# NagsTheProgrammer/WindGNN

Hardware: NVIDIA B200
Metric: gcn_gru_forward_sequences_per_s (higher is better)
Workload: dtype f32

## Files before the change

### windgnn_b200/csrc/abi.cu

```cuda

#include "../../include/windgnn_b200.h"

#include <cmath>
#include <cstdarg>
#include <cstdio>
#include <cstdlib>
#include <cstring>
#include <mutex>
#include <vector>

#include "gcn.cuh"
#include "gcn_bwd.cuh"
#include "gcn_bwd_rows.cuh"
#include "gcn_rows.cuh"
#include "gcn_sparse.cuh"
#include "gcn_sparse_plan.cuh"
#include "gemm_kb.cuh"
#include "gru_bwd.cuh"
#include "inproj.cuh"
#include "inproj_tc2.cuh"
#include "recur.cuh"
#include "recur_tc.cuh"
#include "recur_unit.cuh"
#include "sgemm.cuh"
#include "train_misc.cuh"
#include "wg_common.cuh"

namespace {

thread_local char g_err[512] = "";

int fail(int code, const char* fmt, ...) {
    va_list ap;
    va_start(ap, fmt);
    vsnprintf(g_err, sizeof(g_err), fmt, ap);
    va_end(ap);
    return code;
}

#define WG_CUDA(expr)                                                                          \
    do {                                                                                       \
        cudaError_t e_ = (expr);                                                               \
        if (e_ != cudaSuccess)                                                                 \
            return fail(WG_ERR_CUDA, "%s failed: %s (%s:%d)", #expr, cudaGetErrorString(e_),   \
                        __FILE__, __LINE__);                                                   \
    } while (0)

struct DeviceGuard {
    int prev = -1;
    cudaError_t err = cudaSuccess;
    explicit DeviceGuard(int dev) {
        err = cudaGetDevice(&prev);
        if (err == cudaSuccess && prev != dev) err = cudaSetDevice(dev);
    }
    ~DeviceGuard() {
        int cur = -1;
        if (prev >= 0 && cudaGetDevice(&cur) == cudaSuccess && cur != prev) cudaSetDevice(prev);
    }
};

constexpr size_t kAlign = 256;
size_t align_up(size_t v) { return (v + kAlign - 1) / kAlign * kAlign; }

enum GcnKind { kGcnRows, kGcn13x7, kGcn13x4, kGcn16x4, kGcnSparsePlan, kGcnSparseLanes };
enum RecurKind { kRecurTc, kRecurUnit, kRecurWide };

struct Plan {
    int T, S, Fi, Fh, Fo, H;
    long long chunk;
    int I, G;
    int IP;
    int NPB;
    int GP;
    int KP;
    int NPR;
    int n_bias;
    bool sparse;
    GcnKind gcn;
    size_t gcn_smem;
    int gcn_rb;
    int gcn_threads;
    size_t off_sqw, off_sqsteps, off_sqpairs;
    bool tc;
    wg::Tc2Shape tc2;
    RecurKind recur;
    bool regw;
    bool whu;
    int ru_wpg, ru_ht;
    int ru_rmax;
    int rc_ts;
    size_t rc_smem;
    size_t off_wp, off_bias, off_wht, off_whu, off_bhn, off_u, off_gi, off_z, total;
    size_t off_whh_hi, off_whh_lo;
};

long long default_chunk(long long B, size_t bytes_per_seq) {
    long long c = (long long)wg::kNumSMs * wg::kRcBT;
    const size_t cap = (size_t)6 << 30;
    if ((size_t)c * bytes_per_seq > cap) {
        c = (long long)(cap / bytes_per_seq) / wg::kRcBT * wg::kRcBT;
        if (c < wg::kRcBT) c = wg::kRcBT;
    }
    return B < c ? (B < 1 ? 1 : B) : c;
}

GcnKind dense_gcn_kind(int S, int Fi, int Fh, int Fo) {
    if (Fi == 13 && Fh == 13 && Fo == 13) return wg::ceil_div(S, 7) * 7 <= wg::ceil_div(S, 4) * 4 ? kGcn13x7 : kGcn13x4;
    return kGcn16x4;
}

int dense_gcn_geometry(GcnKind k, int S, int Fi, int Fh, int Fo, int& RB, size_t& smem) {
    const int Fmax = Fi > Fh ? (Fi > Fo ? Fi : Fo) : (Fh > Fo ? Fh : Fo);
    if (Fmax > 16) return fail(WG_ERR_UNSUPPORTED, "GCN feature width %d > 16 is not built into the dense kernel", Fmax);
    const int NSG = wg::ceil_div(S, k == kGcn13x7 ? 7 : 4);
    if (NSG > wg::kGcnThreads)
        return fail(WG_ERR_UNSUPPORTED, "S=%d too large for the dense GCN kernel", S);
    auto smem_of = [&](int rb) {
        const size_t floats = k == kGcn13x7   ? wg::gcn_smem_floats<13, 7>(S, Fmax, rb)
                              : k == kGcn13x4 ? wg::gcn_smem_floats<13, 4>(S, Fmax, rb)
                                              : wg::gcn_smem_floats<16, 4>(S, Fmax, rb);
        return floats * 4;
    };
    RB = wg::kGcnThreads / NSG;
    const int in_cols = S * Fi;
    const int need = (in_cols % 4 == 0) ? 1 : (in_cols % 2 == 0 ? 2 : 4);
    if (RB > need) RB -= RB % need;
    smem = smem_of(RB);
    while (smem > (size_t)wg::kMaxSmemOptin / 3 && RB > 2 * need && RB > 8) {
        RB -= need > (RB + 7) / 8 ? need : (RB + 7) / 8 / need * need;
        smem = smem_of(RB);
    }
    while (smem > (size_t)wg::kMaxSmemOptin && RB > 1) {
        RB = RB / 2;
        smem = smem_of(RB);
    }
    if (smem > (size_t)wg::kMaxSmemOptin)
        return fail(WG_ERR_UNSUPPORTED, "dense GCN needs %zu B of shared memory (S=%d); use the sparse path", smem, S);
    return WG_OK;
}

bool force_legacy() {
    const char* e = getenv("WG_FORCE_LEGACY");
    return e && e[0] == '1';
}

long long forecast_piece_rows(const Plan& p, long long Ttot) {
    const long long r = p.chunk * p.T;
    return r < Ttot ? r : Ttot;
}

int plan_layout(Plan& p, long long B, int T, int S, int Fi, int Fh, int Fo, int H, long long chunk, bool sparse,
                int flags, long long table_rows = 0) {
    if (B < 0 || T <= 0 || S <= 0 || Fi <= 0 || Fh <= 0 || Fo <= 0 || H <= 0 || chunk < 0)
        return fail(WG_ERR_BAD_ARG, "non-positive dimension (B=%lld T=%d S=%d F=%d/%d/%d H=%d chunk=%lld)",
                    B, T, S, Fi, Fh, Fo, H, chunk);
    if ((long long)S * Fo > (1 << 20) || H > (1 << 15))
        return fail(WG_ERR_UNSUPPORTED, "dimension too large (S*F_out=%lld, H=%d)", (long long)S * Fo, H);
    p.T = T; p.S = S; p.Fi = Fi; p.Fh = Fh; p.Fo = Fo; p.H = H;
    p.sparse = sparse;
    if (flags & ~WG_FLAG_TENSOR_CORES) return fail(WG_ERR_BAD_ARG, "unknown flags 0x%x", flags);
    p.I = S * Fo;
    p.G = 3 * H;
    p.tc2 = wg::tc2_shape(p.G, p.I);
    p.tc = (flags & WG_FLAG_TENSOR_CORES) != 0;
    if (p.tc && !p.tc2.ok)
        return fail(WG_ERR_UNSUPPORTED, "tensor-core projection: unsupported gate width 3H = %d", p.G);
    p.IP = p.tc ? p.tc2.KP : wg::round_up(p.I, wg::kIpBK);
    p.NPB = wg::round_up(p.G, wg::kIpBN);
    p.GP = wg::round_up(p.G, 8);
    p.KP = wg::round_up(H, 4);
    p.NPR = wg::recur_np(p.G);
    {
        const size_t per_seq = (size_t)T * ((size_t)p.IP + p.GP + (sparse ? (size_t)S * Fo : 0)) * 4;
        p.chunk = chunk > 0 ? chunk : default_chunk(B, per_seq);
        if (p.chunk > B && B > 0) p.chunk = B;
    }
    if (sparse)
        p.gcn = Fi <= wg::kSpF && Fo <= wg::kSpF && Fh <= wg::kSqMaxFh &&
                        wg::gcn_sparse_plan_smem_bytes(S, Fi, Fo) <= (size_t)wg::kMaxSmemOptin
                    ? kGcnSparsePlan : kGcnSparseLanes;
    else if (wg::gcn_rows_applies(S, Fi, Fh, Fo) && wg::gcn_rows_smem_floats(S) * 4 <= (size_t)wg::kMaxSmemOptin &&
             !force_legacy())
        p.gcn = kGcnRows;
    else
        p.gcn = dense_gcn_kind(S, Fi, Fh, Fo);
    p.whu = wg::recur_u_applies(H);
    if (p.tc && wg::recur_tc_applies(H) && wg::recur_tc_smem_bytes(H) <= (size_t)wg::kMaxSmemOptin)
        p.recur = kRecurTc;
    else if (p.whu && wg::recur_u_smem_floats(H, wg::kRuMinR) * 4 <= (size_t)wg::kMaxSmemOptin)
        p.recur = kRecurUnit;
    else
        p.recur = kRecurWide;
    p.regw = (p.KP == 104 || p.KP == 24) && p.NPR <= wg::kRwThreads &&
             wg::recur_regw_smem_floats(p.KP, p.NPR, p.GP) * 4 <= (size_t)wg::kMaxSmemOptin;
    p.ru_wpg = wg::recur_u_wpg(H);
    p.ru_ht = H == 102 || H == 21 ? H : 0;
    size_t o = 0;
    const int wrows = p.tc && p.tc2.NP > p.NPB ? p.tc2.NP : p.NPB;
    p.n_bias = wrows > 512 ? wrows : 512;
    p.off_wp = o;   o = align_up(o + (p.tc ? wg::tc2_w_halves(p.tc2) * 2 : (size_t)p.NPB * p.IP * 4));
    p.off_bias = o; o = align_up(o + (size_t)p.n_bias * 4);
    p.off_wht = o;  o = align_up(o + (size_t)p.KP * p.NPR * 4);
    p.off_whu = o;
    if (p.whu) o = align_up(o + (size_t)p.KP * 3 * wg::recur_u_hp2(H) * 4);
    p.off_bhn = o;  o = align_up(o + (size_t)p.KP * 4);
    const bool tc_recur = p.recur == kRecurTc;
    p.off_whh_hi = o; if (tc_recur) o = align_up(o + wg::recur_tc_w_halves(H) * 2);
    p.off_whh_lo = o; if (tc_recur) o = align_up(o + wg::recur_tc_w_halves(H) * 2);
    const size_t rows = table_rows > 0 ? (size_t)forecast_piece_rows(p, table_rows) : (size_t)p.chunk * T;
    const size_t rows_tiled = (rows + wg::kUTileRows - 1) / wg::kUTileRows * wg::kUTileRows;
    p.off_u = o;    o = align_up(o + rows_tiled * p.IP * 4);
    const size_t rows_gi =
        table_rows > 0 ? (size_t)table_rows : (size_t)((p.chunk + wg::kRtSeqs - 1) / wg::kRtSeqs * wg::kRtSeqs) * T;
    p.off_gi = o;   o = align_up(o + rows_gi * p.GP * 4);
    p.off_z = o;    if (sparse) o = align_up(o + (rows + wg::kNumSMs) * (size_t)S * Fo * 4);
    const bool sq = p.gcn == kGcnSparsePlan;
    p.off_sqw = o;     if (sq) o = align_up(o + sizeof(wg::SqWeights));
    p.off_sqsteps = o;
    p.off_sqpairs = o + (size_t)wg::round_up(wg::ceil_div(S, 32), 4) * sizeof(int);
    if (sq) o = align_up(o + wg::sq_plan_bytes(S));
    p.total = o;
    return WG_OK;
}

int plan_launch(Plan& p) {
    const long long rows = p.chunk * p.T;
    switch (p.gcn) {
    case kGcnRows:
        p.gcn_smem = wg::gcn_rows_smem_floats(p.S) * 4;
        p.gcn_threads = wg::gcn_rows_warps(p.S) * 32;
        break;
    case kGcnSparsePlan: {
        p.gcn_smem = wg::gcn_sparse_plan_smem_bytes(p.S, p.Fi, p.Fo);
        const long long rt = (rows + wg::kSpThreads - 1) / wg::kSpThreads * wg::kSpThreads;
        if (rt / 32 > 65535) return fail(WG_ERR_UNSUPPORTED, "sparse GCN: chunk of %lld rows too large", rows);
        break;
    }
    case kGcnSparseLanes:
        if (p.Fi > wg::kSpF || p.Fo > wg::kSpF)
            return fail(WG_ERR_UNSUPPORTED, "sparse GCN: F_in / F_out must be <= %d (got %d / %d)", wg::kSpF, p.Fi, p.Fo);
        p.gcn_smem = ((size_t)2 * p.Fh * wg::kSpF + p.Fh) * 4;
        if (p.gcn_smem > (size_t)wg::kMaxSmemOptin)
            return fail(WG_ERR_UNSUPPORTED, "sparse GCN: hidden width %d too large", p.Fh);
        break;
    default: {
        const int rc = dense_gcn_geometry(p.gcn, p.S, p.Fi, p.Fh, p.Fo, p.gcn_rb, p.gcn_smem);
        if (rc) return rc;
    }
    }
    if (!p.tc && (rows + wg::kIpBM - 1) / wg::kIpBM * (p.NPB / wg::kIpBN) > 0x7fffffffLL)
        return fail(WG_ERR_UNSUPPORTED, "projection grid too large");
    if (p.recur == kRecurUnit) {
        p.ru_rmax = wg::kRuMaxR;
        while (p.ru_rmax > wg::kRuMinR && wg::recur_u_smem_floats(p.H, p.ru_rmax) * 4 > (size_t)wg::kMaxSmemOptin)
            --p.ru_rmax;
    } else if (p.recur == kRecurWide) {
        p.rc_ts = wg::recur_stage_steps(p.H);
        p.rc_smem = wg::recur_smem_floats(p.KP, p.GP, p.H, p.rc_ts) * 4;
        if (p.rc_smem > (size_t)wg::kMaxSmemOptin) {
            p.rc_ts = 0;
            p.rc_smem = wg::recur_smem_floats(p.KP, p.GP) * 4;
        }
        if (p.rc_smem > (size_t)wg::kMaxSmemOptin)
            return fail(WG_ERR_UNSUPPORTED, "GRU hidden size %d: state does not fit shared memory", p.H);
    }
    return WG_OK;
}

int make_plan(Plan& p, long long B, int T, int S, int Fi, int Fh, int Fo, int H, long long chunk,
              bool sparse = false, int flags = 0) {
    const int rc = plan_layout(p, B, T, S, Fi, Fh, Fo, H, chunk, sparse, flags);
    return rc ? rc : plan_launch(p);
}

int check_ws(const void* ws, size_t bytes, size_t need) {
    if (!ws) return fail(WG_ERR_WORKSPACE, "workspace is NULL (need %zu bytes)", need);
    if (reinterpret_cast<uintptr_t>(ws) % kAlign)
        return fail(WG_ERR_WORKSPACE, "workspace must be %zu-byte aligned", kAlign);
    if (bytes < need)
        return fail(WG_ERR_WORKSPACE, "workspace too small: %zu bytes given, %zu needed", bytes, need);
    return WG_OK;
}

template <typename T>
T* ws_ptr(void* ws, size_t off) { return reinterpret_cast<T*>(static_cast<char*>(ws) + off); }

__global__ void pack_params_kernel(const float* __restrict__ w_ih, const float* __restrict__ w_hh,
                                   const float* __restrict__ b_ih, const float* __restrict__ b_hh,
                                   float* __restrict__ wp, float* __restrict__ bias,
                                   float* __restrict__ wht, float* __restrict__ whu, float* __restrict__ bhn, int I,
                                   int H, int IP, int NPB, int KP, int NPR, int pack_wih, int n_bias) {
    const int G = 3 * H;
    const long long n_wp = pack_wih ? (long long)NPB * IP : 0;
    const long long n_wht = (long long)KP * NPR;
    const long long stride = (long long)gridDim.x * blockDim.x;
    const long long t0 = (long long)blockIdx.x * blockDim.x + threadIdx.x;
    for (long long e = t0; e < n_wp; e += stride) {
        const int nl = (int)(e % wg::kIpBN);
        const long long r = e / wg::kIpBN;
        const int k = (int)(r % IP), n = (int)(r / IP) * wg::kIpBN + nl;
        wp[e] = (n < G && k < I) ? w_ih[(size_t)n * I + k] : 0.0f;
    }
    for (long long e = t0; e < n_wht; e += stride) {
        const int k = (int)(e / NPR), n = (int)(e % NPR);
        wht[e] = (k < H && n < G) ? w_hh[(size_t)n * H + k] : 0.0f;
    }
    if (whu != nullptr) {
        const int HP2 = wg::recur_u_hp2(H);
        const long long n_whu = (long long)KP * 3 * HP2;
        for (long long e = t0; e < n_whu; e += stride) {
            const int j = (int)(e % HP2);
            const long long r = e / HP2;
            const int g = (int)(r % 3), k = (int)(r / 3);
            whu[e] = (k < H && j < H) ? w_hh[((size_t)g * H + j) * H + k] : 0.0f;
        }
    }
    for (long long e = t0; e < n_bias; e += stride) {
        float v = 0.0f;
        if (e < G) v = b_ih[e] + (e < 2 * H ? b_hh[e] : 0.0f);
        bias[e] = v;
    }
    for (long long e = t0; e < KP; e += stride) bhn[e] = e < H ? b_hh[2 * H + e] : 0.0f;
}

template <int FP, int SG, bool EXACT, int LAYERS, bool TILED>
int launch_gcn_t(const float* X, const float* adj, const float* W1, const float* b1, const float* W2,
                 const float* b2, float* out, long long R, int S, int Fi, int Fh, int Fo, int ldo, int RB, size_t smem,
                 cudaStream_t st) {
    auto kern = wg::gcn_kernel<FP, SG, EXACT, LAYERS, TILED>;
    WG_CUDA(cudaFuncSetAttribute(kern, cudaFuncAttributeMaxDynamicSharedMemorySize, (int)smem));
    int per_sm = 0;
    WG_CUDA(cudaOccupancyMaxActiveBlocksPerMultiprocessor(&per_sm, kern, wg::kGcnThreads, smem));
    if (per_sm < 1) per_sm = 1;
    const long long nblocks = (R + RB - 1) / RB;
    long long grid = (long long)wg::kNumSMs * per_sm;
    if (grid > nblocks) grid = nblocks;
    if (grid < 1) return WG_OK;
    kern<<<(unsigned)grid, wg::kGcnThreads, smem, st>>>(X, adj, W1, b1, W2, b2, out, R, S, Fi, Fh, Fo, ldo, RB);
    WG_CUDA(cudaGetLastError());
    return WG_OK;
}

template <int LAYERS, bool TILED>
int launch_gcn_dense(GcnKind k, int RB, size_t smem, const float* X, const float* adj, const float* W1,
                     const float* b1, const float* W2, const float* b2, float* out, long long R, int S, int Fi, int Fh,
                     int Fo, int ldo, cudaStream_t st) {
#define WG_GCN(FP, SG, EX) \
    launch_gcn_t<FP, SG, EX, LAYERS, TILED>(X, adj, W1, b1, W2, b2, out, R, S, Fi, Fh, Fo, ldo, RB, smem, st)
    if (k == kGcn13x7) return WG_GCN(13, 7, true);
    if (k == kGcn13x4) return WG_GCN(13, 4, true);
    return WG_GCN(16, 4, false);
#undef WG_GCN
}

int launch_gcn_rows(const Plan& p, const float* X, const float* adj, const float* W1, const float* b1,
                    const float* W2, const float* b2, float* out, long long R, cudaStream_t st) {
    WG_CUDA(cudaFuncSetAttribute(wg::gcn_rows_kernel, cudaFuncAttributeMaxDynamicSharedMemorySize, (int)p.gcn_smem));
    int per_sm = 0;
    WG_CUDA(cudaOccupancyMaxActiveBlocksPerMultiprocessor(&per_sm, wg::gcn_rows_kernel, p.gcn_threads, p.gcn_smem));
    if (per_sm < 1) per_sm = 1;
    const long long nblocks = (R + wg::kGrRows - 1) / wg::kGrRows;
    long long grid = (long long)wg::kNumSMs * per_sm;
    if (grid > nblocks) grid = nblocks;
    if (grid < 1) return WG_OK;
    wg::gcn_rows_kernel<<<(unsigned)grid, p.gcn_threads, p.gcn_smem, st>>>(X, adj, W1, b1, W2, b2, out, R, p.S, p.IP);
    WG_CUDA(cudaGetLastError());
    return WG_OK;
}

struct Graph {
    const float* adj;
    const int* rowptr;
    const int* colidx;
    const float* vals;
};

int launch_gcn_sparse(const Plan& p, void* ws, const Graph& g, const float* x, const float* w1, const float* b1,
                      const float* w2, const float* b2, long long rows, cudaStream_t st) {
    if (rows < 1) return WG_OK;
    if (p.gcn == kGcnSparsePlan) {
        const bool narrow = p.Fi <= 13 && p.Fo <= 13, exact = p.Fi == 13 && p.Fo == 13;
        auto kern = exact ? wg::gcn_sparse_plan_kernel<13, true>
                          : narrow ? wg::gcn_sparse_plan_kernel<13, false> : wg::gcn_sparse_plan_kernel<16, false>;
        WG_CUDA(cudaFuncSetAttribute(kern, cudaFuncAttributeMaxDynamicSharedMemorySize, (int)p.gcn_smem));
        const unsigned grid = (unsigned)(rows < wg::kNumSMs ? rows : wg::kNumSMs);
        float* urow = ws_ptr<float>(ws, p.off_z);
        float* zscr = urow + (size_t)rows * p.S * p.Fo;
        kern<<<grid, wg::kSqThreads, p.gcn_smem, st>>>(x, g.rowptr, g.colidx, g.vals, ws_ptr<int>(ws, p.off_sqsteps),
                                                       ws_ptr<int2>(ws, p.off_sqpairs), zscr, urow, rows, p.S, p.Fi,
                                                       p.Fh, p.Fo);
        WG_CUDA(cudaGetLastError());
        const long long rt = (rows + wg::kSpThreads - 1) / wg::kSpThreads * wg::kSpThreads;
        const dim3 tg((unsigned)((p.S + 31) / 32), (unsigned)(rt / 32));
        const size_t tsmem = wg::fmajor_to_tiles_smem_bytes(p.Fo);
        WG_CUDA(cudaFuncSetAttribute(wg::fmajor_to_tiles_kernel, cudaFuncAttributeMaxDynamicSharedMemorySize, (int)tsmem));
        wg::fmajor_to_tiles_kernel<<<tg, 256, tsmem, st>>>(urow, ws_ptr<float>(ws, p.off_u), rows, p.S, p.Fo, p.IP);
        WG_CUDA(cudaGetLastError());
        return WG_OK;
    }
    const long long tiles = (rows + wg::kSpThreads - 1) / wg::kSpThreads;
    int chunks = (int)((4LL * wg::kNumSMs * 4 + tiles - 1) / tiles);
    if (chunks < 1) chunks = 1;
    if (chunks > p.S) chunks = p.S;
    const int s_chunk = (p.S + chunks - 1) / chunks;
    const dim3 grid((unsigned)tiles, (unsigned)((p.S + s_chunk - 1) / s_chunk));
    WG_CUDA(cudaFuncSetAttribute(wg::gcn_sparse_l1_kernel, cudaFuncAttributeMaxDynamicSharedMemorySize,
                                 (int)p.gcn_smem));
    wg::gcn_sparse_l1_kernel<<<grid, wg::kSpThreads, p.gcn_smem, st>>>(x, g.rowptr, g.colidx, g.vals, w1, b1, w2,
                                                                       ws_ptr<float>(ws, p.off_z), rows, p.S, p.Fi,
                                                                       p.Fh, p.Fo, s_chunk);
    WG_CUDA(cudaGetLastError());
    wg::gcn_sparse_l2_kernel<<<grid, wg::kSpThreads, 0, st>>>(ws_ptr<float>(ws, p.off_z), g.rowptr, g.colidx, g.vals,
                                                             b2, ws_ptr<float>(ws, p.off_u), rows, p.S, p.Fo, p.IP,
                                                             s_chunk);
    WG_CUDA(cudaGetLastError());
    return WG_OK;
}

int launch_gcn(const Plan& p, void* ws, const Graph& g, const float* x, const float* w1, const float* b1,
               const float* w2, const float* b2, long long rows, cudaStream_t st) {
    float* u = ws_ptr<float>(ws, p.off_u);
    if (p.gcn == kGcnRows) return launch_gcn_rows(p, x, g.adj, w1, b1, w2, b2, u, rows, st);
    if (p.sparse) return launch_gcn_sparse(p, ws, g, x, w1, b1, w2, b2, rows, st);
    return launch_gcn_dense<2, true>(p.gcn, p.gcn_rb, p.gcn_smem, x, g.adj, w1, b1, w2, b2, u, rows, p.S, p.Fi, p.Fh,
                                     p.Fo, p.IP, st);
}

int launch_inproj_tc(const Plan& p, void* ws, long long rows, cudaStream_t st, float* gi) {
    const long long m_tiles = (rows + wg::kT2BM - 1) / wg::kT2BM;
    if (m_tiles < 1) return WG_OK;
    const wg::Tc2Shape& t = p.tc2;
    WG_CUDA(cudaFuncSetAttribute(wg::inproj_tc2_kernel, cudaFuncAttributeMaxDynamicSharedMemorySize,
                                 (int)t.smem_bytes));
    const long long tiles = m_tiles * t.n_nt;
    const unsigned grid = (unsigned)(tiles < wg::kNumSMs ? tiles : wg::kNumSMs);
    wg::inproj_tc2_kernel<<<grid, wg::kT2Threads, t.smem_bytes, st>>>(
        ws_ptr<float>(ws, p.off_u), ws_ptr<__half>(ws, p.off_wp), ws_ptr<float>(ws, p.off_bias), gi, rows, p.IP,
        t.KP, p.GP, t.n_nt, t.N_each, t.stages);
    WG_CUDA(cudaGetLastError());
    return WG_OK;
}

int launch_inproj(const Plan& p, void* ws, long long rows, cudaStream_t st, float* gi) {
    if (p.tc) return launch_inproj_tc(p, ws, rows, st, gi);
    const long long m_tiles = (rows + wg::kIpBM - 1) / wg::kIpBM;
    const int n_tiles = p.NPB / wg::kIpBN;
    const long long grid = m_tiles * n_tiles;
    if (grid < 1) return WG_OK;
    WG_CUDA(cudaFuncSetAttribute(wg::inproj_kernel, cudaFuncAttributeMaxDynamicSharedMemorySize,
                                 wg::kIpSmemBytes));
    wg::inproj_kernel<<<(unsigned)grid, wg::kIpThreads, wg::kIpSmemBytes, st>>>(
        ws_ptr<float>(ws, p.off_u), ws_ptr<float>(ws, p.off_wp), ws_ptr<float>(ws, p.off_bias), gi, rows, p.IP, p.GP,
        n_tiles);
    WG_CUDA(cudaGetLastError());
    return WG_OK;
}


int launch_recur_wide(const Plan& p, void* ws, float* out, long long Bc, cudaStream_t st, const long long* row0) {
    auto kern = row0 ? wg::gru_recur_kernel<true> : wg::gru_recur_kernel<false>;
    WG_CUDA(cudaFuncSetAttribute(kern, cudaFuncAttributeMaxDynamicSharedMemorySize, (int)p.rc_smem));
    const long long grid = (Bc + wg::kRcBT - 1) / wg::kRcBT;
    if (grid < 1) return WG_OK;
    kern<<<(unsigned)grid, wg::kRcWarps * 32, p.rc_smem, st>>>(ws_ptr<float>(ws, p.off_gi), ws_ptr<float>(ws, p.off_wht),
                                                              ws_ptr<float>(ws, p.off_bhn), out, Bc, p.T, p.H, p.GP,
                                                              p.KP, p.NPR, row0 ? 0 : p.rc_ts, row0);
    WG_CUDA(cudaGetLastError());
    return WG_OK;
}

int recur_u_pick_r(long long Bc, int ngrp) {
    int best = wg::kRuMaxR;
    long long best_cost = -1;
    for (int r = wg::kRuMaxR; r >= wg::kRuMinR; --r) {
        const long long ctas = (Bc + (long long)ngrp * r - 1) / ((long long)ngrp * r);
        const long long waves = (ctas + wg::kNumSMs - 1) / wg::kNumSMs;
        const long long cost = waves * (r + 1);
        if (best_cost < 0 || cost < best_cost) { best_cost = cost; best = r; }
    }
    return best;
}

using RegwKernel = decltype(&wg::gru_recur_regw_kernel<false, 1, 24>);
template <bool SAVE, int KPT, bool WIN = false>
RegwKernel regw_kernel(int nb) {
    const RegwKernel k[4] = {wg::gru_recur_regw_kernel<SAVE, 1, KPT, WIN>, wg::gru_recur_regw_kernel<SAVE, 2, KPT, WIN>,
                             wg::gru_recur_regw_kernel<SAVE, 3, KPT, WIN>, wg::gru_recur_regw_kernel<SAVE, 4, KPT, WIN>};
    return k[nb - 1];
}
int launch_recur_regw(const Plan& p, void* ws, float* out, long long Bc, int nb, cudaStream_t st, float* gsave,
                      int ldsave, const long long* row0) {
    if (Bc < 1) return WG_OK;
    const RegwKernel kern =
        row0    ? (p.KP == 104 ? regw_kernel<false, 104, true>(nb) : regw_kernel<false, 24, true>(nb))
        : gsave ? (p.KP == 104 ? regw_kernel<true, 104>(nb) : regw_kernel<true, 24>(nb))
                : (p.KP == 104 ? regw_kernel<false, 104>(nb) : regw_kernel<false, 24>(nb));
    const size_t smem = wg::recur_regw_smem_floats(p.KP, p.NPR, p.GP) * 4;
    WG_CUDA(cudaFuncSetAttribute(kern, cudaFuncAttributeMaxDynamicSharedMemorySize, (int)smem));
    const long long grid = (Bc + wg::kRsBT - 1) / wg::kRsBT;
    kern<<<(unsigned)grid, wg::kRwThreads, smem, st>>>(ws_ptr<float>(ws, p.off_gi), ws_ptr<float>(ws, p.off_wht),
                                                      ws_ptr<float>(ws, p.off_bhn), out, Bc, p.T, p.H, p.GP, p.NPR,
                                                      gsave, ldsave, row0);
    WG_CUDA(cudaGetLastError());
    return WG_OK;
}

using UnitKernel = decltype(&wg::gru_recur_unit_kernel<4, 1, false, 0>);
template <int WPG, bool SAVE, int HT, bool WIN>
UnitKernel unit_kernel(int r) {
    const UnitKernel k[5] = {
        wg::gru_recur_unit_kernel<4, WPG, SAVE, HT, WIN>, wg::gru_recur_unit_kernel<5, WPG, SAVE, HT, WIN>,
        wg::gru_recur_unit_kernel<6, WPG, SAVE, HT, WIN>, wg::gru_recur_unit_kernel<7, WPG, SAVE, HT, WIN>,
        wg::gru_recur_unit_kernel<8, WPG, SAVE, HT, WIN>};
    return k[r - wg::kRuMinR];
}
template <bool SAVE, bool WIN = false>
UnitKernel unit_kernel(const Plan& p, int r) {
    if (p.ru_ht == 102) return unit_kernel<2, SAVE, 102, WIN>(r);
    if (p.ru_ht == 21) return unit_kernel<1, SAVE, 21, WIN>(r);
    return p.ru_wpg == 1 ? unit_kernel<1, SAVE, 0, WIN>(r) : unit_kernel<2, SAVE, 0, WIN>(r);
}
int launch_recur_unit(const Plan& p, void* ws, float* out, long long Bc, int r, cudaStream_t st, float* gsave,
                      int ldsave, const long long* row0) {
    const UnitKernel kern =
        row0 ? unit_kernel<false, true>(p, r) : gsave ? unit_kernel<true>(p, r) : unit_kernel<false>(p, r);
    const size_t smem = wg::recur_u_smem_floats(p.H, r) * 4;
    WG_CUDA(cudaFuncSetAttribute(kern, cudaFuncAttributeMaxDynamicSharedMemorySize, (int)smem));
    const int per_cta = (wg::kRuWarps / p.ru_wpg) * r;
    const long long grid = (Bc + per_cta - 1) / per_cta;
    if (grid < 1) return WG_OK;
    const int handover = p.ru_wpg == 1 ? 1 : 0;
    kern<<<(unsigned)grid, wg::kRuThreads, smem, st>>>(ws_ptr<float>(ws, p.off_gi), ws_ptr<float>(ws, p.off_whu),
                                                      ws_ptr<float>(ws, p.off_bhn), out, Bc, p.T, p.H, gsave, ldsave,
                                                      handover, row0);
    WG_CUDA(cudaGetLastError());
    return WG_OK;
}

int launch_recur_tc(const Plan& p, void* ws, float* out, long long Bc, cudaStream_t st, const long long* row0) {
    auto kern = row0 ? wg::gru_recur_tc_kernel<true> : wg::gru_recur_tc_kernel<false>;
    const size_t smem = wg::recur_tc_smem_bytes(p.H);
    WG_CUDA(cudaFuncSetAttribute(kern, cudaFuncAttributeMaxDynamicSharedMemorySize, (int)smem));
    const long long grid = (Bc + wg::kRtSeqs - 1) / wg::kRtSeqs;
    if (grid < 1) return WG_OK;
    kern<<<(unsigned)grid, wg::kRtThreads, smem, st>>>(ws_ptr<float>(ws, p.off_gi), ws_ptr<__half>(ws, p.off_whh_hi),
                                                      ws_ptr<__half>(ws, p.off_whh_lo), ws_ptr<float>(ws, p.off_bhn),
                                                      out, Bc, p.T, p.H, p.GP, row0);
    WG_CUDA(cudaGetLastError());
    return WG_OK;
}

bool regw_serves(const Plan& p, long long Bc) {
    return p.recur != kRecurTc && p.regw && Bc <= 2LL * wg::kRsBT * wg::kNumSMs;
}

int launch_recur(const Plan& p, void* ws, float* out, long long Bc, cudaStream_t st, float* gsave, int ldsave,
                 const long long* row0 = nullptr) {
    if (regw_serves(p, Bc)) return launch_recur_regw(p, ws, out, Bc, Bc >= 4 ? 4 : (int)Bc, st, gsave, ldsave, row0);
    if (p.recur == kRecurUnit) {
        const int r = recur_u_pick_r(Bc, wg::kRuWarps / p.ru_wpg);
        return launch_recur_unit(p, ws, out, Bc, r < p.ru_rmax ? r : p.ru_rmax, st, gsave, ldsave, row0);
    }
    if (p.recur == kRecurTc) return launch_recur_tc(p, ws, out, Bc, st, row0);
    return launch_recur_wide(p, ws, out, Bc, st, row0);
}

int launch_pack(const Plan& p, void* ws, const float* w_ih, const float* w_hh, const float* b_ih,
                const float* b_hh, cudaStream_t st) {
    pack_params_kernel<<<wg::kNumSMs * 2, 256, 0, st>>>(
        w_ih, w_hh, b_ih, b_hh, ws_ptr<float>(ws, p.off_wp), ws_ptr<float>(ws, p.off_bias),
        ws_ptr<float>(ws, p.off_wht), p.whu ? ws_ptr<float>(ws, p.off_whu) : nullptr, ws_ptr<float>(ws, p.off_bhn),
        p.I, p.H, p.IP, p.NPB, p.KP, p.NPR, p.tc ? 0 : 1, p.n_bias);
    WG_CUDA(cudaGetLastError());
    if (p.tc) {
        wg::pack_wih_tc2_kernel<<<wg::kNumSMs * 2, 256, 0, st>>>(w_ih, ws_ptr<__half>(ws, p.off_wp), p.G, p.I, p.tc2.KP,
                                                                p.tc2.n_nt, p.tc2.N_each);
        WG_CUDA(cudaGetLastError());
    }
    if (p.recur == kRecurTc) {
        wg::pack_whh_tc_kernel<<<wg::kNumSMs, 256, 0, st>>>(w_hh, ws_ptr<__half>(ws, p.off_whh_hi),
                                                           ws_ptr<__half>(ws, p.off_whh_lo), p.H);
        WG_CUDA(cudaGetLastError());
    }
    return WG_OK;
}

int run_chunk(const Plan& p, void* ws, const Graph& g, const float* x, const float* w1, const float* b1,
              const float* w2, const float* b2, float* out, long long Bc, cudaStream_t st, float* gsave = nullptr,
              int ldsave = 0) {
    const long long rows = Bc * p.T;
    int rc = launch_gcn(p, ws, g, x, w1, b1, w2, b2, rows, st);
    if (rc) return rc;
    rc = launch_inproj(p, ws, rows, st, ws_ptr<float>(ws, p.off_gi));
    if (rc) return rc;
    return launch_recur(p, ws, out, Bc, st, gsave, ldsave);
}

constexpr int kMaxDevices = 64;

std::mutex g_sq_mu;
struct SqDeviceState { cudaEvent_t ev = nullptr; cudaStream_t last = nullptr; bool recorded = false; };
SqDeviceState g_sq_dev[kMaxDevices];

int prepare_sparse(const Plan& p, void* ws, const Graph& g, const float* w1, const float* b1, const float* w2,
                   const float* b2, int device, cudaStream_t st) {
    if (device >= kMaxDevices) return fail(WG_ERR_BAD_ARG, "device index %d out of range", device);
    wg::SqWeights* stage = ws_ptr<wg::SqWeights>(ws, p.off_sqw);
    wg::sq_pack_weights_kernel<<<32, 256, 0, st>>>(w1, b1, w2, b2, stage, p.Fi, p.Fh, p.Fo);
    WG_CUDA(cudaGetLastError());
    const int wbs = wg::ceil_div(p.S, 32);
    wg::csr_plan_kernel<<<wg::ceil_div(wbs, 4), 128, 0, st>>>(g.rowptr, g.colidx, g.vals, p.S,
                                                             ws_ptr<int>(ws, p.off_sqsteps),
                                                             ws_ptr<int2>(ws, p.off_sqpairs));
    WG_CUDA(cudaGetLastError());
    SqDeviceState& d = g_sq_dev[device];
    cudaStreamCaptureStatus cap = cudaStreamCaptureStatusNone;
    cudaStreamIsCapturing(st, &cap);
    if (cap == cudaStreamCaptureStatusNone && d.recorded && d.last != st) WG_CUDA(cudaStreamWaitEvent(st, d.ev, 0));
    WG_CUDA(cudaMemcpyToSymbolAsync(wg::c_sq, stage, sizeof(wg::SqWeights), 0, cudaMemcpyDeviceToDevice, st));
    return WG_OK;
}
int finish_sparse(int device, cudaStream_t st) {
    SqDeviceState& d = g_sq_dev[device];
    cudaStreamCaptureStatus cap = cudaStreamCaptureStatusNone;
    cudaStreamIsCapturing(st, &cap);
    if (cap != cudaStreamCaptureStatusNone) return WG_OK;
    if (!d.ev) WG_CUDA(cudaEventCreateWithFlags(&d.ev, cudaEventDisableTiming));
    WG_CUDA(cudaEventRecord(d.ev, st));
    d.last = st;
    d.recorded = true;
    return WG_OK;
}

bool any_null(std::initializer_list<const void*> ps) {
    for (const void* q : ps)
        if (!q) return true;
    return false;
}

template <typename Stages>
int run_packed(const Plan& p, size_t need, const Graph& g, const float* x, const float* w1, const float* b1,
               const float* w2, const float* b2, const float* w_ih, const float* w_hh, const float* b_ih,
               const float* b_hh, const float* out, void* ws, size_t ws_bytes, int device, void* stream,
               Stages stages) {
    const bool no_graph = p.sparse ? any_null({g.rowptr, g.colidx, g.vals}) : !g.adj;
    if (no_graph || any_null({x, w1, b1, w2, b2, w_ih, w_hh, b_ih, b_hh, out}))
        return fail(WG_ERR_BAD_ARG, "null pointer argument");
    int rc = check_ws(ws, ws_bytes, need);
    if (rc) return rc;
    DeviceGuard dg(device);
    WG_CUDA(dg.err);
    cudaStream_t st = static_cast<cudaStream_t>(stream);
    if ((rc = launch_pack(p, ws, w_ih, w_hh, b_ih, b_hh, st))) return rc;
    const bool sq = p.gcn == kGcnSparsePlan;
    std::unique_lock<std::mutex> sq_lock(g_sq_mu, std::defer_lock);
    if (sq) {
        sq_lock.lock();
        if ((rc = prepare_sparse(p, ws, g, w1, b1, w2, b2, device, st))) return rc;
    }
    if ((rc = stages(st))) return rc;
    return sq ? finish_sparse(device, st) : WG_OK;
}

int forward(const Plan& p, size_t need, const Graph& g, const float* x, const float* w1, const float* b1,
            const float* w2, const float* b2, const float* w_ih, const float* w_hh, const float* b_ih,
            const float* b_hh, float* out, long long B, void* ws, size_t ws_bytes, int device, void* stream,
            float* gsave = nullptr, int ldsave = 0) {
    if (B == 0) return WG_OK;
    auto stages = [&](cudaStream_t st) {
        const size_t x_seq = (size_t)p.T * p.S * p.Fi, o_seq = (size_t)p.T * p.H;
        for (long long b0 = 0; b0 < B; b0 += p.chunk) {
            const long long Bc = (B - b0) < p.chunk ? (B - b0) : p.chunk;
            const int rc = run_chunk(p, ws, g, x + (size_t)b0 * x_seq, w1, b1, w2, b2, out + (size_t)b0 * o_seq, Bc,
                                     st, gsave ? gsave + (size_t)b0 * p.T * ldsave : nullptr, ldsave);
            if (rc) return rc;
        }
        return (int)WG_OK;
    };
    return run_packed(p, need, g, x, w1, b1, w2, b2, w_ih, w_hh, b_ih, b_hh, out, ws, ws_bytes, device, stream,
                      stages);
}

struct ForecastPlan {
    Plan p;
    size_t off_row0, total;
};

int make_forecast_plan(ForecastPlan& f, long long N, long long Ttot, int L, int S, int Fi, int Fh, int Fo, int H,
                       long long chunk, bool sparse, int flags) {
    if (N < 0 || L < 1 || Ttot < L)
        return fail(WG_ERR_BAD_ARG, "forecast: need N >= 0 and 1 <= L <= Ttot (N=%lld L=%d Ttot=%lld)", N, L, Ttot);
    int rc = plan_layout(f.p, N, L, S, Fi, Fh, Fo, H, chunk, sparse, flags, Ttot);
    if (rc || (rc = plan_launch(f.p))) return rc;
    f.off_row0 = f.p.total;
    f.total = align_up(f.off_row0 + (size_t)N * sizeof(long long));
    return WG_OK;
}

int forecast(const ForecastPlan& f, const Graph& g, const float* table, const int64_t* starts, const float* w1,
             const float* b1, const float* w2, const float* b2, const float* w_ih, const float* w_hh,
             const float* b_ih, const float* b_hh, float* out, long long N, long long Ttot, void* ws,
             size_t ws_bytes, int device, void* stream) {
    const Plan& p = f.p;
    if (N == 0) return WG_OK;
    if (!starts) return fail(WG_ERR_BAD_ARG, "starts is NULL (N=%lld)", N);
    const long long last = Ttot - p.T;
    long long lo = 0, hi = 0;
    for (long long n = 0; n < N; ++n) {
        const long long s = starts[n];
        if (s < 0 || s > last)
            return fail(WG_ERR_BAD_ARG, "starts[%lld] = %lld outside [0, Ttot - L] = [0, %lld]", n, s, last);
        if (n == 0 || s < lo) lo = s;
        if (n == 0 || s > hi) hi = s;
    }
    auto stages = [&](cudaStream_t st) {
        std::vector<long long> row0((size_t)N);
        for (long long n = 0; n < N; ++n) row0[(size_t)n] = starts[n] - lo;
        long long* row0_dev = ws_ptr<long long>(ws, f.off_row0);
        WG_CUDA(cudaMemcpyAsync(row0_dev, row0.data(), (size_t)N * sizeof(long long), cudaMemcpyHostToDevice, st));
        float* gi = ws_ptr<float>(ws, p.off_gi);
        const size_t x_row = (size_t)p.S * p.Fi;
        const long long span = hi + p.T - lo, piece = forecast_piece_rows(p, Ttot);
        for (long long r0 = 0; r0 < span; r0 += piece) {
            const long long rows = span - r0 < piece ? span - r0 : piece;
            int rc = launch_gcn(p, ws, g, table + (size_t)(lo + r0) * x_row, w1, b1, w2, b2, rows, st);
            if (rc || (rc = launch_inproj(p, ws, rows, st, gi + (size_t)r0 * p.GP))) return rc;
        }
        for (long long b0 = 0; b0 < N; b0 += p.chunk) {
            const long long Bc = (N - b0) < p.chunk ? (N - b0) : p.chunk;
            const int rc = launch_recur(p, ws, out + (size_t)b0 * p.H, Bc, st, nullptr, 0, row0_dev + b0);
            if (rc) return rc;
        }
        return (int)WG_OK;
    };
    return run_packed(p, f.total, g, table, w1, b1, w2, b2, w_ih, w_hh, b_ih, b_hh, out, ws, ws_bytes, device, stream,
                      stages);
}

template <typename Launch>
int run_stage(long long Bc, int T, int S, int Fi, int Fh, int Fo, int H, long long chunk, int flags, void* ws,
              size_t ws_bytes, int device, void* stream, Launch launch) {
    Plan p;
    int rc = make_plan(p, chunk, T, S, Fi, Fh, Fo, H, chunk, false, flags);
    if (rc) return rc;
    if (Bc < 0 || Bc > p.chunk) return fail(WG_ERR_BAD_ARG, "Bc=%lld outside [0, chunk=%lld]", Bc, p.chunk);
    if ((rc = check_ws(ws, ws_bytes, p.total))) return rc;
    DeviceGuard g(device);
    WG_CUDA(g.err);
    return launch(p, static_cast<cudaStream_t>(stream));
}


__global__ void pack_wih_bwd_kernel(const float* __restrict__ w_ih, float* __restrict__ wp, float* __restrict__ zb,
                                    int G, int I, int KP, int NP) {
    const long long total = (long long)NP * KP;
    for (long long e = (long long)blockIdx.x * blockDim.x + threadIdx.x; e < total;
         e += (long long)gridDim.x * blockDim.x) {
        const int nl = (int)(e % wg::kIpBN);
        const long long r = e / wg::kIpBN;
        const int k = (int)(r % KP), n = (int)(r / KP) * wg::kIpBN + nl;
        wp[e] = (k < G && n < I) ? w_ih[(size_t)k * I + n] : 0.0f;
    }
    for (int e = blockIdx.x * blockDim.x + threadIdx.x; e < NP; e += gridDim.x * blockDim.x) zb[e] = 0.0f;
}

using GbRegwKernel = decltype(&wg::gru_bwd_regw_kernel<4, 24>);
using GbKernel = decltype(&wg::gru_bwd_kernel<4>);
constexpr int kGbRegwBT[4] = {4, 8, 16, 28};
template <int HPT>
GbRegwKernel gb_regw_kernel(int i) {
    const GbRegwKernel k[4] = {wg::gru_bwd_regw_kernel<4, HPT>, wg::gru_bwd_regw_kernel<8, HPT>,
                               wg::gru_bwd_regw_kernel<16, HPT>, wg::gru_bwd_regw_kernel<28, HPT>};
    return k[i];
}

enum GcnBwdKind { kGcnBwdRows, kGcnBwd13, kGcnBwd16 };

struct TrainPlan {
    Plan f;
    int LD4;
    long long rows;
    GbRegwKernel gb_regw;
    GbKernel gb;
    int HP, GR;
    int gb_threads, gb_grid, gb_parts;
    size_t gb_smem;
    int splits_hh_a, splits_hh_b;
    int mt_ih, nt_ih, splits_ih;
    long long kt_per_ih;
    int ldu, KPd, NPd;
    dim3 tg_du;
    long long mt_du;
    int nt_du;
    GcnBwdKind gcn;
    int grid_gcn, rb_gcn, parts_gcn;
    size_t smem_gcn;
    size_t off_gates, off_dg, off_dgt, off_wpb, off_zb, off_du, off_biasp, off_gcnp, off_splitk, total;
};

int pick_splits(long long M, long long N, long long K) {
    const long long tiles = ((M + wg::kSgBM - 1) / wg::kSgBM) * ((N + wg::kSgBN - 1) / wg::kSgBN);
    long long s = (2LL * wg::kNumSMs) / tiles;
    const long long kmax = (K + 63) / 64;
    if (s > kmax) s = kmax;
    return s < 1 ? 1 : (int)s;
}

size_t param_count(int S, int Fi, int Fh, int Fo, int H) {
    const size_t I = (size_t)S * Fo, G = 3 * (size_t)H;
    return (size_t)Fi * Fh + Fh + (size_t)Fh * Fo + Fo + G * I + G * H + G + G;
}

constexpr int kTrainMaxH = 106;

int make_train_plan(TrainPlan& tp, long long B, int T, int S, int Fi, int Fh, int Fo, int H) {
    const long long Bn = B > 0 ? B : 1;
    int rc = plan_layout(tp.f, B, T, S, Fi, Fh, Fo, H, Bn, false, 0);
    if (rc) return rc;
    const Plan& p = tp.f;
    if (Fi > 16 || Fh > 16 || Fo > 16)
        return fail(WG_ERR_UNSUPPORTED, "training: GCN feature widths must be <= 16 (got %d / %d / %d)", Fi, Fh, Fo);
    tp.LD4 = wg::round_up(4 * H, 4);
    tp.HP = wg::round_up(H, 4);
    int bt;
    if (tp.HP == 104 || tp.HP == 24) {
        int i = 0;
        while (i < 3 && (Bn + kGbRegwBT[i] - 1) / kGbRegwBT[i] > wg::kNumSMs) ++i;
        bt = kGbRegwBT[i];
        tp.gb_regw = tp.HP == 104 ? gb_regw_kernel<104>(i) : gb_regw_kernel<24>(i);
        tp.gb = nullptr;
        tp.gb_threads = wg::kGrwThreads;
        tp.gb_smem = wg::gru_bwd_regw_smem_floats(tp.HP, bt) * 4;
    } else {
        bt = Bn > 4LL * wg::kNumSMs ? wg::kGbBT : 4;
        tp.GR = wg::gru_bwd_gr(H, bt);
        tp.gb_smem = wg::gru_bwd_smem_floats(tp.HP, tp.GR, bt) * 4;
        if (tp.HP > 128 || (tp.HP / 4) * (bt / 4) * wg::gru_bwd_ksplit(bt) > wg::kGbThreads ||
            tp.gb_smem > (size_t)wg::kMaxSmemOptin)
            return fail(WG_ERR_UNSUPPORTED, "training: GRU hidden size %d too large for the shared-memory BPTT kernel", H);
        tp.gb_regw = nullptr;
        tp.gb = bt == 4 ? wg::gru_bwd_kernel<4> : wg::gru_bwd_kernel<wg::kGbBT>;
        tp.gb_threads = wg::kGbThreads;
    }
    tp.gb_grid = (int)((Bn + bt - 1) / bt);
    tp.gb_parts = tp.gb_grid * (tp.gb_regw ? 3 : 2);
    if (H > kTrainMaxH || !(regw_serves(p, B) || p.recur == kRecurUnit))
        return fail(WG_ERR_UNSUPPORTED, "training: GRU hidden size %d does not fit the shared-memory recurrence", H);
    tp.rows = Bn * T;
    tp.ldu = wg::round_up(p.I, 4);
    tp.KPd = wg::round_up(p.G, wg::kIpBK);
    tp.NPd = wg::round_up(p.I, wg::kIpBN);
    if (wg::gcn_bwd_rows_applies(S, Fi, Fh, Fo) &&
        wg::gcn_bwd_rows_smem_floats(S, tp.ldu) * 4 <= (size_t)wg::kMaxSmemOptin) {
        tp.gcn = kGcnBwdRows;
        tp.rb_gcn = wg::kGb2Rows;
        tp.smem_gcn = wg::gcn_bwd_rows_smem_floats(S, tp.ldu) * 4;
        const long long nblk = (tp.rows + wg::kGb2Rows - 1) / wg::kGb2Rows;
        const int per_sm = tp.smem_gcn + 1024 <= (size_t)(228 * 1024) / 2 ? 2 : 1;
        tp.grid_gcn = (int)(nblk < (long long)per_sm * wg::kNumSMs ? nblk : (long long)per_sm * wg::kNumSMs);
        tp.parts_gcn = tp.grid_gcn * wg::kGb2Slices;
    } else {
        tp.gcn = Fi == 13 && Fh == 13 && Fo == 13 ? kGcnBwd13 : kGcnBwd16;
        const int NSG = wg::ceil_div(S, wg::kGbwSG);
        if (NSG > wg::kGcnThreads) return fail(WG_ERR_UNSUPPORTED, "training: S=%d too large for the dense GCN kernels", S);
        int RB = wg::kGbwThreads / NSG;
        const int cols = S * Fi;
        const int need = (cols % 4 == 0) ? 1 : (cols % 2 == 0) ? 2 : 4;
        if (RB > need) RB -= RB % need;
        auto smem_of = [&](int rb) { return wg::gcn_bwd_smem_floats(S, tp.ldu, rb) * 4; };
        while (smem_of(RB) > (size_t)wg::kMaxSmemOptin && RB > 1) RB = (RB > need) ? RB - need : RB - 1;
        if (smem_of(RB) > (size_t)wg::kMaxSmemOptin)
            return fail(WG_ERR_UNSUPPORTED, "training: S=%d does not fit the shared-memory GCN backward", S);
        tp.rb_gcn = RB;
        tp.smem_gcn = smem_of(RB);
        const long long nblk = (tp.rows + RB - 1) / RB;
// ... 578 lines not shown
```

### windgnn_b200/csrc/inproj.cuh

```cuda
#pragma once

#include "wg_common.cuh"

namespace wg {

constexpr int kIpBM = 128;
constexpr int kIpBN = 64;
constexpr int kIpBK = 16;
constexpr int kIpStages = 4;
constexpr int kIpThreads = 128;
constexpr int kIpStageFloats = kIpBK * (kIpBM + kIpBN);
constexpr int kIpStageBytes = kIpStageFloats * 4;
constexpr int kIpSmemBytes = kIpStages * kIpStageBytes + 64;

__global__ void __launch_bounds__(kIpThreads, 4)
    inproj_kernel(const float* __restrict__ At, const float* __restrict__ Bt,
                  const float* __restrict__ bias, float* __restrict__ C, long long M, int K, int ldc,
                  int n_tiles) {
    extern __shared__ __align__(128) unsigned char smem_raw[];
    float* stage0 = reinterpret_cast<float*>(smem_raw);
    uint64_t* bars = reinterpret_cast<uint64_t*>(smem_raw + kIpStages * kIpStageBytes);

    const int tid = threadIdx.x;
    const long long tile = blockIdx.x;
    const int nt = (int)(tile % n_tiles);
    const long long mt = tile / n_tiles;
    const int KT = K / kIpBK;
    const float* a_src = At + (size_t)mt * K * kIpBM;
    const float* b_src = Bt + (size_t)nt * K * kIpBN;

    if (tid == 0) {
#pragma unroll
        for (int s = 0; s < kIpStages; ++s) mbar_init(&bars[s], 1);
        fence_mbar_init();
    }
    __syncthreads();

    auto issue = [&](int kt) {
        const int slot = kt % kIpStages;
        float* dst = stage0 + slot * kIpStageFloats;
        mbar_expect_tx(&bars[slot], kIpStageBytes);
        bulk_g2s(dst, a_src + (size_t)kt * kIpBK * kIpBM, kIpBK * kIpBM * 4, &bars[slot]);
        bulk_g2s(dst + kIpBK * kIpBM, b_src + (size_t)kt * kIpBK * kIpBN, kIpBK * kIpBN * 4, &bars[slot]);
    };
    if (tid == 0) {
#pragma unroll
        for (int s = 0; s < kIpStages - 1; ++s)
            if (s < KT) issue(s);
    }

    const int ty = tid >> 3;
    const int tx = tid & 7;

    float2 acc[8][4];
#pragma unroll
    for (int i = 0; i < 8; ++i)
#pragma unroll
        for (int j = 0; j < 4; ++j) acc[i][j] = make_float2(0.0f, 0.0f);

    for (int kt = 0; kt < KT; ++kt) {
        __syncthreads();
        if (tid == 0 && kt + kIpStages - 1 < KT) issue(kt + kIpStages - 1);
        const int slot = kt % kIpStages;
        mbar_wait(&bars[slot], (kt / kIpStages) & 1);
        const float* as = stage0 + slot * kIpStageFloats + ty * 4;
        const float* bs = stage0 + slot * kIpStageFloats + kIpBK * kIpBM + tx * 4;
#pragma unroll
        for (int k = 0; k < kIpBK; ++k) {
            const float4 a0 = *reinterpret_cast<const float4*>(as + k * kIpBM);
            const float4 a1 = *reinterpret_cast<const float4*>(as + k * kIpBM + 64);
            const float4 b0 = *reinterpret_cast<const float4*>(bs + k * kIpBN);
            const float4 b1 = *reinterpret_cast<const float4*>(bs + k * kIpBN + 32);
            const float av[8] = {a0.x, a0.y, a0.z, a0.w, a1.x, a1.y, a1.z, a1.w};
            const float2 bp[4] = {make_float2(b0.x, b0.y), make_float2(b0.z, b0.w),
                                  make_float2(b1.x, b1.y), make_float2(b1.z, b1.w)};
#pragma unroll
            for (int i = 0; i < 8; ++i) {
                const float2 aa = make_float2(av[i], av[i]);
#pragma unroll
                for (int j = 0; j < 4; ++j) acc[i][j] = __ffma2_rn(aa, bp[j], acc[i][j]);
            }
        }
    }

    const int n0 = nt * kIpBN;
    const float4 bia0 = __ldg(reinterpret_cast<const float4*>(bias + n0 + tx * 4));
    const float4 bia1 = __ldg(reinterpret_cast<const float4*>(bias + n0 + 32 + tx * 4));
    const long long m0 = mt * kIpBM;
#pragma unroll
    for (int i = 0; i < 8; ++i) {
        const long long gm = m0 + (i < 4 ? ty * 4 + i : 64 + ty * 4 + (i - 4));
        if (gm < M) {
            float* crow = C + (size_t)gm * ldc;
            const int c0 = n0 + tx * 4, c1 = n0 + 32 + tx * 4;
            if (c0 < ldc)
                *reinterpret_cast<float4*>(crow + c0) = make_float4(
                    acc[i][0].x + bia0.x, acc[i][0].y + bia0.y, acc[i][1].x + bia0.z, acc[i][1].y + bia0.w);
            if (c1 < ldc)
                *reinterpret_cast<float4*>(crow + c1) = make_float4(
                    acc[i][2].x + bia1.x, acc[i][2].y + bia1.y, acc[i][3].x + bia1.z, acc[i][3].y + bia1.w);
        }
    }
}

}
```

Measured before the change: 777,100.

## Add persistent wide-N input projection kernel covering all gate columns per tile

```diff
diff --git a/windgnn_b200/csrc/abi.cu b/windgnn_b200/csrc/abi.cu
--- a/windgnn_b200/csrc/abi.cu
+++ b/windgnn_b200/csrc/abi.cu
@@ -71,6 +71,10 @@
     int I, G;
     int IP;
     int NPB;
+    bool ip_wide;
+    int ip_bn;
+    int ip_threads;
+    size_t ip_smem;
     int GP;
     int KP;
     int NPR;
@@ -167,6 +171,8 @@
         return fail(WG_ERR_UNSUPPORTED, "tensor-core projection: unsupported gate width 3H = %d", p.G);
     p.IP = p.tc ? p.tc2.KP : wg::round_up(p.I, wg::kIpBK);
     p.NPB = wg::round_up(p.G, wg::kIpBN);
+    p.ip_wide = !p.tc && p.NPB == wg::kIwBN;
+    p.ip_bn = p.ip_wide ? wg::kIwBN : wg::kIpBN;
     p.GP = wg::round_up(p.G, 8);
     p.KP = wg::round_up(H, 4);
     p.NPR = wg::recur_np(p.G);
@@ -248,8 +254,12 @@
         if (rc) return rc;
     }
     }
-    if (!p.tc && (rows + wg::kIpBM - 1) / wg::kIpBM * (p.NPB / wg::kIpBN) > 0x7fffffffLL)
-        return fail(WG_ERR_UNSUPPORTED, "projection grid too large");
+    if (!p.tc) {
+        p.ip_threads = p.ip_wide ? wg::kIwThreads : wg::kIpThreads;
+        p.ip_smem = p.ip_wide ? wg::kIwSmemBytes : wg::kIpSmemBytes;
+        if ((rows + wg::kIpBM - 1) / wg::kIpBM * (p.NPB / p.ip_bn) > 0x7fffffffLL)
+            return fail(WG_ERR_UNSUPPORTED, "projection grid too large");
+    }
     if (p.recur == kRecurUnit) {
         p.ru_rmax = wg::kRuMaxR;
         while (p.ru_rmax > wg::kRuMinR && wg::recur_u_smem_floats(p.H, p.ru_rmax) * 4 > (size_t)wg::kMaxSmemOptin)
@@ -289,16 +299,16 @@
                                    const float* __restrict__ b_ih, const float* __restrict__ b_hh,
                                    float* __restrict__ wp, float* __restrict__ bias,
                                    float* __restrict__ wht, float* __restrict__ whu, float* __restrict__ bhn, int I,
-                                   int H, int IP, int NPB, int KP, int NPR, int pack_wih, int n_bias) {
+                                   int H, int IP, int NPB, int BN, int KP, int NPR, int pack_wih, int n_bias) {
     const int G = 3 * H;
     const long long n_wp = pack_wih ? (long long)NPB * IP : 0;
     const long long n_wht = (long long)KP * NPR;
     const long long stride = (long long)gridDim.x * blockDim.x;
     const long long t0 = (long long)blockIdx.x * blockDim.x + threadIdx.x;
     for (long long e = t0; e < n_wp; e += stride) {
-        const int nl = (int)(e % wg::kIpBN);
-        const long long r = e / wg::kIpBN;
-        const int k = (int)(r % IP), n = (int)(r / IP) * wg::kIpBN + nl;
+        const int nl = (int)(e % BN);
+        const long long r = e / BN;
+        const int k = (int)(r % IP), n = (int)(r / IP) * BN + nl;
         wp[e] = (n < G && k < I) ? w_ih[(size_t)n * I + k] : 0.0f;
     }
     for (long long e = t0; e < n_wht; e += stride) {
@@ -444,14 +454,21 @@
 int launch_inproj(const Plan& p, void* ws, long long rows, cudaStream_t st, float* gi) {
     if (p.tc) return launch_inproj_tc(p, ws, rows, st, gi);
     const long long m_tiles = (rows + wg::kIpBM - 1) / wg::kIpBM;
-    const int n_tiles = p.NPB / wg::kIpBN;
-    const long long grid = m_tiles * n_tiles;
-    if (grid < 1) return WG_OK;
-    WG_CUDA(cudaFuncSetAttribute(wg::inproj_kernel, cudaFuncAttributeMaxDynamicSharedMemorySize,
-                                 wg::kIpSmemBytes));
-    wg::inproj_kernel<<<(unsigned)grid, wg::kIpThreads, wg::kIpSmemBytes, st>>>(
-        ws_ptr<float>(ws, p.off_u), ws_ptr<float>(ws, p.off_wp), ws_ptr<float>(ws, p.off_bias), gi, rows, p.IP, p.GP,
-        n_tiles);
+    if (m_tiles < 1) return WG_OK;
+    const float* u = ws_ptr<float>(ws, p.off_u);
+    const float* wp = ws_ptr<float>(ws, p.off_wp);
+    const float* bias = ws_ptr<float>(ws, p.off_bias);
+    if (p.ip_wide) {
+        WG_CUDA(cudaFuncSetAttribute(wg::inproj_wide_kernel, cudaFuncAttributeMaxDynamicSharedMemorySize,
+                                     (int)p.ip_smem));
+        const unsigned grid = (unsigned)(m_tiles < wg::kNumSMs ? m_tiles : wg::kNumSMs);
+        wg::inproj_wide_kernel<<<grid, p.ip_threads, p.ip_smem, st>>>(u, wp, bias, gi, rows, p.IP, p.GP);
+    } else {
+        const int n_tiles = p.NPB / wg::kIpBN;
+        WG_CUDA(cudaFuncSetAttribute(wg::inproj_kernel, cudaFuncAttributeMaxDynamicSharedMemorySize, (int)p.ip_smem));
+        wg::inproj_kernel<<<(unsigned)(m_tiles * n_tiles), p.ip_threads, p.ip_smem, st>>>(u, wp, bias, gi, rows, p.IP,
+                                                                                          p.GP, n_tiles);
+    }
     WG_CUDA(cudaGetLastError());
     return WG_OK;
 }
@@ -570,7 +587,7 @@
     pack_params_kernel<<<wg::kNumSMs * 2, 256, 0, st>>>(
         w_ih, w_hh, b_ih, b_hh, ws_ptr<float>(ws, p.off_wp), ws_ptr<float>(ws, p.off_bias),
         ws_ptr<float>(ws, p.off_wht), p.whu ? ws_ptr<float>(ws, p.off_whu) : nullptr, ws_ptr<float>(ws, p.off_bhn),
-        p.I, p.H, p.IP, p.NPB, p.KP, p.NPR, p.tc ? 0 : 1, p.n_bias);
+        p.I, p.H, p.IP, p.NPB, p.ip_bn, p.KP, p.NPR, p.tc ? 0 : 1, p.n_bias);
     WG_CUDA(cudaGetLastError());
     if (p.tc) {
         wg::pack_wih_tc2_kernel<<<wg::kNumSMs * 2, 256, 0, st>>>(w_ih, ws_ptr<__half>(ws, p.off_wp), p.G, p.I, p.tc2.KP,
diff --git a/windgnn_b200/csrc/inproj.cuh b/windgnn_b200/csrc/inproj.cuh
--- a/windgnn_b200/csrc/inproj.cuh
+++ b/windgnn_b200/csrc/inproj.cuh
@@ -103,4 +103,104 @@
     }
 }
 
+constexpr int kIwBN = 320;
+constexpr int kIwThreads = 256;
+constexpr int kIwStages = 4;
+constexpr int kIwStageFloats = kIpBK * (kIpBM + kIwBN);
+constexpr int kIwStageBytes = kIwStageFloats * 4;
+constexpr int kIwSmemBytes = kIwStages * kIwStageBytes + 64;
+
+__global__ void __launch_bounds__(kIwThreads, 1)
+    inproj_wide_kernel(const float* __restrict__ At, const float* __restrict__ Bt,
+                       const float* __restrict__ bias, float* __restrict__ C, long long M, int K, int ldc) {
+    extern __shared__ __align__(128) unsigned char smem_raw[];
+    float* stage0 = reinterpret_cast<float*>(smem_raw);
+    uint64_t* bars = reinterpret_cast<uint64_t*>(smem_raw + kIwStages * kIwStageBytes);
+
+    const int tid = threadIdx.x;
+    const int KT = K / kIpBK;
+    const int m_tiles = (int)((M + kIpBM - 1) / kIpBM);
+
+    if (tid == 0) {
+#pragma unroll
+        for (int s = 0; s < kIwStages; ++s) mbar_init(&bars[s], 1);
+        fence_mbar_init();
+    }
+    __syncthreads();
+
+    auto issue = [&](int mt, int kt, int slot) {
+        while (kt >= KT) { kt -= KT; mt += gridDim.x; }
+        if (mt >= m_tiles) return;
+        float* dst = stage0 + slot * kIwStageFloats;
+        mbar_expect_tx(&bars[slot], kIwStageBytes);
+        bulk_g2s(dst, At + ((size_t)mt * K + (size_t)kt * kIpBK) * kIpBM, kIpBK * kIpBM * 4, &bars[slot]);
+        bulk_g2s(dst + kIpBK * kIpBM, Bt + (size_t)kt * kIpBK * kIwBN, kIpBK * kIwBN * 4, &bars[slot]);
+    };
+    if (tid == 0) {
+#pragma unroll
+        for (int s = 0; s < kIwStages - 1; ++s) issue(blockIdx.x, s, s);
+    }
+
+    const int ty = tid >> 4;
+    const int tx = tid & 15;
+    int slot = 0;
+    unsigned phase = 0;
+
+    for (int mt = blockIdx.x; mt < m_tiles; mt += gridDim.x) {
+        float2 acc[8][10];
+#pragma unroll
+        for (int i = 0; i < 8; ++i)
+#pragma unroll
+            for (int j = 0; j < 10; ++j) acc[i][j] = make_float2(0.0f, 0.0f);
+
+        for (int kt = 0; kt < KT; ++kt) {
+            __syncthreads();
+            if (tid == 0) issue(mt, kt + kIwStages - 1, slot == 0 ? kIwStages - 1 : slot - 1);
+            mbar_wait(&bars[slot], phase);
+            const float* as = stage0 + slot * kIwStageFloats + ty * 4;
+            const float* bs = stage0 + slot * kIwStageFloats + kIpBK * kIpBM + tx * 20;
+#pragma unroll
+            for (int k = 0; k < kIpBK; ++k) {
+                const float4 a0 = *reinterpret_cast<const float4*>(as + k * kIpBM);
+                const float4 a1 = *reinterpret_cast<const float4*>(as + k * kIpBM + 64);
+                float2 bp[10];
+#pragma unroll
+                for (int q = 0; q < 5; ++q) {
+                    const float4 b = *reinterpret_cast<const float4*>(bs + k * kIwBN + q * 4);
+                    bp[2 * q] = make_float2(b.x, b.y);
+                    bp[2 * q + 1] = make_float2(b.z, b.w);
+                }
+                const float av[8] = {a0.x, a0.y, a0.z, a0.w, a1.x, a1.y, a1.z, a1.w};
+#pragma unroll
+                for (int i = 0; i < 8; ++i) {
+                    const float2 aa = make_float2(av[i], av[i]);
+#pragma unroll
+                    for (int j = 0; j < 10; ++j) acc[i][j] = __ffma2_rn(aa, bp[j], acc[i][j]);
+                }
+            }
+            if (++slot == kIwStages) { slot = 0; phase ^= 1; }
+        }
+
+        const long long m0 = mt * kIpBM;
+        const int c0 = tx * 20;
+#pragma unroll
+        for (int i = 0; i < 8; ++i) {
+            const long long gm = m0 + (i < 4 ? ty * 4 + i : 64 + ty * 4 + (i - 4));
+            if (gm < M) {
+                float* crow = C + (size_t)gm * ldc;
+#pragma unroll
+                for (int q = 0; q < 5; ++q) {
+                    const int c = c0 + q * 4;
+                    if (c < ldc) {
+                        const float4 b = __ldg(reinterpret_cast<const float4*>(bias + c));
+                        *reinterpret_cast<float4*>(crow + c) =
+                            make_float4(acc[i][2 * q].x + b.x, acc[i][2 * q].y + b.y, acc[i][2 * q + 1].x + b.z,
+                                        acc[i][2 * q + 1].y + b.w);
+                    }
+                }
+            }
+        }
+    }
 }
+
+}
```

After: 716,100 (median of 6 runs). 0.921x the previous value.
